# imironhead/ml_super_resolution

Hardware: AMD Instinct MI355X
Metric: VDSR-20 training patches/sec (41x41, batch 256 per GPU); fwd HR megapixels/sec alongside (higher is better)
Workload: dtype f32; 1 GPU; BASELINE configs[2]: VDSR 20-layer 3x3x64 residual, RGB, batch 256x41x41 per GPU, fwd+bwd+TF-Adam, random-init weights; global_batch=256, patch=41, parallelism=dp1

## Files before the change

### ml_super_resolution_amd/csrc/conv_narrow.hip

```cpp
#include "launchers.h"
namespace srx {
typedef float f32x3 __attribute__((ext_vector_type(3)));
typedef unsigned u32x3v __attribute__((ext_vector_type(3)));

template <int CTRL>
__device__ __forceinline__ float dpp_add(float v) {
    const int moved = __builtin_amdgcn_update_dpp(0, __float_as_int(v), CTRL, 0xf, 0xf, false);
    return v + __int_as_float(moved);
}

struct PixWalk {
    int n, oh, ow;
    __device__ __forceinline__ void init(unsigned p, int OH, int OW) {
        const unsigned t = p / (unsigned)OW;
        ow = (int)(p - t * (unsigned)OW);
        n = (int)(t / (unsigned)OH);
        oh = (int)(t - (unsigned)n * (unsigned)OH);
    }
    __device__ __forceinline__ void step16(int OH, int OW) { step(16, OH, OW); }
    __device__ __forceinline__ void step(int d, int OH, int OW) {
        ow += d;
        while (ow >= OW) {
            ow -= OW;
            oh += 1;
            if (oh == OH) { oh = 0; n += 1; }
        }
    }
};
template <int KH, int KW>
__device__ __forceinline__ void tap_offsets(int (&off)[KH * KW], const PixWalk& q, bool live, int H, int W, int pad_t, int pad_l,
                                            int PB, int lane_b) {
    const int centre = ((q.n * H + q.oh - pad_t) * W + (q.ow - pad_l)) * PB + lane_b;
    bool rok[KH], cok[KW];
#pragma unroll
    for (int kh = 0; kh < KH; ++kh) rok[kh] = live && (unsigned)(q.oh + kh - pad_t) < (unsigned)H;
#pragma unroll
    for (int kw = 0; kw < KW; ++kw) cok[kw] = (unsigned)(q.ow + kw - pad_l) < (unsigned)W;
#pragma unroll
    for (int kh = 0; kh < KH; ++kh)
#pragma unroll
        for (int kw = 0; kw < KW; ++kw)
            off[kh * KW + kw] = (rok[kh] && cok[kw]) ? centre + (kh * W + kw) * PB : kOobOffset;
}

template <int KH, int KW, int CIN, int CO>
__global__ __launch_bounds__(256) void conv_narrow_kernel(const ConvArgs a, long total_px, int iters) {
    static_assert(CIN == 64, "16 lanes x 4 channels per pixel");
    constexpr int TAPS = KH * KW;
    const int c4 = threadIdx.x & 15;
    const int sub = threadIdx.x >> 4;
    float wr[TAPS][4][CO];
#pragma unroll
    for (int t = 0; t < TAPS; ++t)
#pragma unroll
        for (int e = 0; e < 4; ++e)
#pragma unroll
            for (int c = 0; c < CO; ++c) wr[t][e][c] = a.w[((size_t)t * CIN + 4 * c4 + e) * CO + c];
    float bias[CO];
#pragma unroll
    for (int c = 0; c < CO; ++c) bias[c] = a.bias ? a.bias[c] : 0.0f;
    const __amdgpu_buffer_rsrc_t xrs = __builtin_amdgcn_make_buffer_rsrc(const_cast<float*>(a.x), 0,
                                                                         a.N * a.H * a.W * CIN * 4, 0x00020000);
    const unsigned p0 = blockIdx.x * (unsigned)iters * 16u + sub;
    PixWalk q;
    q.init(p0 < (unsigned)total_px ? p0 : 0u, a.OH, a.OW);
    for (int it = 0; it < iters; ++it, q.step16(a.OH, a.OW)) {
        const unsigned p = p0 + (unsigned)it * 16u;
        const bool live = p < (unsigned)total_px;
        int off[TAPS];
        tap_offsets<KH, KW>(off, q, live, a.H, a.W, a.pad_t, a.pad_l, CIN * 4, 16 * c4);
        f32x4 v[TAPS];
#pragma unroll
        for (int tp = 0; tp < TAPS; ++tp)
            v[tp] = __builtin_bit_cast(f32x4, __builtin_amdgcn_raw_buffer_load_b128(xrs, off[tp], 0, 0));
        float acc[CO];
#pragma unroll
        for (int c = 0; c < CO; ++c) acc[c] = 0.0f;
#pragma unroll
        for (int tp = 0; tp < TAPS; ++tp)
#pragma unroll
            for (int e = 0; e < 4; ++e)
#pragma unroll
                for (int c = 0; c < CO; ++c) acc[c] = fmaf(v[tp][e], wr[tp][e][c], acc[c]);
#pragma unroll
        for (int c = 0; c < CO; ++c) {
            float r = acc[c];
            r = dpp_add<0xB1>(r);
            r = dpp_add<0x4E>(r);
            r = dpp_add<0x124>(r);
            r = dpp_add<0x128>(r);
            acc[c] = r;
        }
        if (live && c4 < CO) {
            float r = (c4 == 0) ? acc[0] : (c4 == 1 ? acc[1 < CO ? 1 : 0] : acc[2 < CO ? 2 : 0]);
            r = act_apply(r + ((c4 == 0) ? bias[0] : (c4 == 1 ? bias[1 < CO ? 1 : 0] : bias[2 < CO ? 2 : 0])), a.act);
            const size_t o = (size_t)p * CO + c4;
            if (a.skip) r += a.skip[o];
            if (a.post_relu) r = act_apply(r, a.post_relu);
            a.y[o] = r;
        }
    }
}

template <int KH, int KW, bool NOUT, int CW = 64>
__global__ __launch_bounds__(256) void wgrad_narrow_kernel(const WgradArgs a, long total_px, int iters) {
    constexpr int TAPS = KH * KW, CN = 3;
    constexpr int LPP = CW / 4;
    constexpr int PPI = 256 / LPP;
    constexpr int NB = NOUT ? CN : 4;
    constexpr int NV = TAPS * 4 * CN + NB;
    __shared__ float red[4 * NV * LPP];
    const int c4 = threadIdx.x & (LPP - 1);
    const int sub = threadIdx.x / LPP;
    const int wave = threadIdx.x >> 6;
    float acc[NV];
#pragma unroll
    for (int i = 0; i < NV; ++i) acc[i] = 0.0f;
    const __amdgpu_buffer_rsrc_t xrs = __builtin_amdgcn_make_buffer_rsrc(
        const_cast<float*>(a.x), 0, a.N * a.H * a.W * (NOUT ? CW : CN) * 4, 0x00020000);
    const __amdgpu_buffer_rsrc_t drs = __builtin_amdgcn_make_buffer_rsrc(
        const_cast<float*>(a.dpre), 0, a.N * a.OH * a.OW * (NOUT ? CN : CW) * 4, 0x00020000);
    const unsigned p0 = blockIdx.x * (unsigned)iters * (unsigned)PPI + sub;
    PixWalk q;
    q.init(p0 < (unsigned)total_px ? p0 : 0u, a.OH, a.OW);
    for (int it = 0; it < iters; ++it, q.step(PPI, a.OH, a.OW)) {
        const unsigned p = p0 + (unsigned)it * (unsigned)PPI;
        const bool live = p < (unsigned)total_px;
        int off[TAPS];
        tap_offsets<KH, KW>(off, q, live, a.H, a.W, a.pad_t, a.pad_l, (NOUT ? CW : CN) * 4, NOUT ? 16 * c4 : 0);
        if constexpr (NOUT) {
            const f32x3 d = __builtin_bit_cast(f32x3, __builtin_amdgcn_raw_buffer_load_b96(drs, live ? (int)(p * CN * 4) : kOobOffset, 0, 0));
            f32x4 v[TAPS];
#pragma unroll
            for (int tp = 0; tp < TAPS; ++tp)
                v[tp] = __builtin_bit_cast(f32x4, __builtin_amdgcn_raw_buffer_load_b128(xrs, off[tp], 0, 0));
#pragma unroll
            for (int tp = 0; tp < TAPS; ++tp)
#pragma unroll
                for (int e = 0; e < 4; ++e)
#pragma unroll
                    for (int c = 0; c < CN; ++c) acc[(tp * 4 + e) * CN + c] = fmaf(v[tp][e], d[c], acc[(tp * 4 + e) * CN + c]);
#pragma unroll
            for (int c = 0; c < CN; ++c) acc[TAPS * 4 * CN + c] += d[c];
        } else {
            const f32x4 d = __builtin_bit_cast(f32x4, __builtin_amdgcn_raw_buffer_load_b128(
                drs, live ? (int)((p * CW + 4 * c4) * 4) : kOobOffset, 0, 0));
            f32x3 v[TAPS];
#pragma unroll
            for (int tp = 0; tp < TAPS; ++tp)
                v[tp] = __builtin_bit_cast(f32x3, __builtin_amdgcn_raw_buffer_load_b96(xrs, off[tp], 0, 0));
#pragma unroll
            for (int tp = 0; tp < TAPS; ++tp)
#pragma unroll
                for (int cn = 0; cn < CN; ++cn)
#pragma unroll
                    for (int e = 0; e < 4; ++e) acc[(tp * CN + cn) * 4 + e] = fmaf(v[tp][cn], d[e], acc[(tp * CN + cn) * 4 + e]);
#pragma unroll
            for (int e = 0; e < 4; ++e) acc[TAPS * 4 * CN + e] += d[e];
        }
    }
#pragma unroll
    for (int i = 0; i < NV; ++i) {
        float r = acc[i];
#pragma unroll
        for (int o = LPP; o < 64; o <<= 1) r += __shfl_xor(r, o);
        if (sub % (64 / LPP) == 0) red[(wave * NV + i) * LPP + c4] = r;
    }
    __syncthreads();
    float* part = a.part + (size_t)blockIdx.x * a.part_stride;
    const int wn = TAPS * CW * CN;
    for (int q = threadIdx.x; q < NV * LPP; q += 256) {
        const int i = q / LPP, l = q % LPP;
        const float r = (red[(0 * NV + i) * LPP + l] + red[(1 * NV + i) * LPP + l]) +
                        (red[(2 * NV + i) * LPP + l] + red[(3 * NV + i) * LPP + l]);
        if (i < TAPS * 4 * CN) {
            int idx;
            if constexpr (NOUT) {
                const int c = i % CN, te = i / CN, e = te & 3, tp = te >> 2;
                idx = (tp * CW + 4 * l + e) * CN + c;
            } else {
                const int e = i & 3, tc = i >> 2;
                idx = tc * CW + 4 * l + e;
            }
            part[idx] = r;
        } else {
            const int b = i - TAPS * 4 * CN;
            if constexpr (NOUT) {
                if (l == 0) part[wn + b] = r;
            } else {
                part[wn + 4 * l + b] = r;
            }
        }
    }
}

bool launch_wgrad_narrow(const ConvKey& k, const WgradArgs& a, int grid, hipStream_t s, hipError_t* err) {
    if (k.kh != 3 || k.kw != 3) return false;
    const bool nout = a.Cin == 64 && a.Cout == 3, nin = a.Cin == 3 && a.Cout == 64, nin32 = a.Cin == 3 && a.Cout == 32;
    if (!nout && !nin && !nin32) return false;
    const long total = (long)a.N * a.OH * a.OW;
    if (total >= (1L << 31) - 4096 || (long)a.N * a.H * a.W * 64 * 4 >= (1L << 31) - 4096 || total * 64 * 4 >= (1L << 31) - 4096)
        return false;
    const long ppi = nin32 ? 32 : 16;
    const int iters = (int)((total + ppi * grid - 1) / (ppi * grid));
    if (nout)
        hipLaunchKernelGGL((wgrad_narrow_kernel<3, 3, true>), dim3(grid), dim3(256), 0, s, a, total, iters);
    else if (nin)
        hipLaunchKernelGGL((wgrad_narrow_kernel<3, 3, false>), dim3(grid), dim3(256), 0, s, a, total, iters);
    else
        hipLaunchKernelGGL((wgrad_narrow_kernel<3, 3, false, 32>), dim3(grid), dim3(256), 0, s, a, total, iters);
    *err = hipGetLastError();
    return true;
}

bool launch_conv_narrow(const ConvKey& k, const ConvArgs& a, hipStream_t s, hipError_t* err) {
    if (k.wt || a.Cout != 3 || a.mask) return false;
    if ((long)a.N * a.H * a.W * a.Cin * 4 >= (1L << 31) - 4096) return false;
    const long total = (long)a.N * a.OH * a.OW;
    int iters = 16;
    while (iters > 1 && total / (16L * iters) < 2048) iters >>= 1;
    const long blocks = (total + 16L * iters - 1) / (16L * iters);
    if (total >= (1L << 31) - 4096) return false;
    if (k.kh == 3 && k.kw == 3 && a.Cin == 64) {
        hipLaunchKernelGGL((conv_narrow_kernel<3, 3, 64, 3>), dim3((unsigned)blocks), dim3(256), 0, s, a, total, iters);
    } else {
        return false;
    }
    *err = hipGetLastError();
    return true;
}
}
```

Before: 20200 patches/s.

## Add sliding-column walk kernel for narrow-channel 3x3 weight gradients

```diff
diff --git a/ml_super_resolution_amd/csrc/conv_narrow.hip b/ml_super_resolution_amd/csrc/conv_narrow.hip
--- a/ml_super_resolution_amd/csrc/conv_narrow.hip
+++ b/ml_super_resolution_amd/csrc/conv_narrow.hip
@@ -1,4 +1,5 @@
 #include "launchers.h"
+#include "narrow_walk.h"
 namespace srx {
 typedef float f32x3 __attribute__((ext_vector_type(3)));
 typedef unsigned u32x3v __attribute__((ext_vector_type(3)));
@@ -102,6 +103,53 @@
     }
 }
 
+template <int KH, int KW, bool NOUT, int CW, bool CE = false>
+__device__ __forceinline__ void wgrad_narrow_close(float (&acc)[KH * KW * 4 * 3 + (NOUT ? 3 : 4)], const WgradArgs& a, float* red) {
+    constexpr int TAPS = KH * KW, CN = 3;
+    constexpr int LPP = CW / 4;
+    constexpr int NB = NOUT ? CN : 4;
+    constexpr int NV = TAPS * 4 * CN + NB;
+    const int c4 = threadIdx.x & (LPP - 1);
+    const int sub = threadIdx.x / LPP;
+    const int wave = threadIdx.x >> 6;
+#pragma unroll
+    for (int i = 0; i < NV; ++i) {
+        float r = acc[i];
+#pragma unroll
+        for (int o = LPP; o < 64; o <<= 1) r += __shfl_xor(r, o);
+        if (sub % (64 / LPP) == 0) red[(wave * NV + i) * LPP + c4] = r;
+    }
+    __syncthreads();
+    float* part = a.part + (size_t)blockIdx.x * a.part_stride;
+    const int wn = TAPS * CW * CN;
+    for (int q = threadIdx.x; q < NV * LPP; q += 256) {
+        const int i = q / LPP, l = q % LPP;
+        const float r = (red[(0 * NV + i) * LPP + l] + red[(1 * NV + i) * LPP + l]) +
+                        (red[(2 * NV + i) * LPP + l] + red[(3 * NV + i) * LPP + l]);
+        if (i < TAPS * 4 * CN) {
+            int idx;
+            if constexpr (NOUT && CE) {
+                const int e = i & 3, tc = i >> 2, c = tc % CN, tp = tc / CN;
+                idx = (tp * CW + 4 * l + e) * CN + c;
+            } else if constexpr (NOUT) {
+                const int c = i % CN, te = i / CN, e = te & 3, tp = te >> 2;
+                idx = (tp * CW + 4 * l + e) * CN + c;
+            } else {
+                const int e = i & 3, tc = i >> 2;
+                idx = tc * CW + 4 * l + e;
+            }
+            part[idx] = r;
+        } else {
+            const int b = i - TAPS * 4 * CN;
+            if constexpr (NOUT) {
+                if (l == 0) part[wn + b] = r;
+            } else {
+                part[wn + 4 * l + b] = r;
+            }
+        }
+    }
+}
+
 template <int KH, int KW, bool NOUT, int CW = 64>
 __global__ __launch_bounds__(256) void wgrad_narrow_kernel(const WgradArgs a, long total_px, int iters) {
     constexpr int TAPS = KH * KW, CN = 3;
@@ -112,7 +160,6 @@
     __shared__ float red[4 * NV * LPP];
     const int c4 = threadIdx.x & (LPP - 1);
     const int sub = threadIdx.x / LPP;
-    const int wave = threadIdx.x >> 6;
     float acc[NV];
 #pragma unroll
     for (int i = 0; i < NV; ++i) acc[i] = 0.0f;
@@ -159,39 +206,116 @@
             for (int e = 0; e < 4; ++e) acc[TAPS * 4 * CN + e] += d[e];
         }
     }
-#pragma unroll
-    for (int i = 0; i < NV; ++i) {
-        float r = acc[i];
-#pragma unroll
-        for (int o = LPP; o < 64; o <<= 1) r += __shfl_xor(r, o);
-        if (sub % (64 / LPP) == 0) red[(wave * NV + i) * LPP + c4] = r;
-    }
-    __syncthreads();
-    float* part = a.part + (size_t)blockIdx.x * a.part_stride;
-    const int wn = TAPS * CW * CN;
-    for (int q = threadIdx.x; q < NV * LPP; q += 256) {
-        const int i = q / LPP, l = q % LPP;
-        const float r = (red[(0 * NV + i) * LPP + l] + red[(1 * NV + i) * LPP + l]) +
-                        (red[(2 * NV + i) * LPP + l] + red[(3 * NV + i) * LPP + l]);
-        if (i < TAPS * 4 * CN) {
-            int idx;
+    wgrad_narrow_close<KH, KW, NOUT, CW>(acc, a, red);
+}
+
+#ifndef SRX_WGRAD_WALK_DEPTH_OUT
+#define SRX_WGRAD_WALK_DEPTH_OUT 2
+#endif
+#ifndef SRX_WGRAD_WALK_DEPTH_IN
+#define SRX_WGRAD_WALK_DEPTH_IN 1
+#endif
+constexpr int kWalkDepthOut = SRX_WGRAD_WALK_DEPTH_OUT, kWalkDepthIn = SRX_WGRAD_WALK_DEPTH_IN;
+template <bool NOUT, int D, int PAD>
+__global__ __launch_bounds__(256, 2) void wgrad_narrow_walk_kernel(const WgradArgs a, unsigned total, int iters) {
+    constexpr int KH = 3, KW = 3, TAPS = KH * KW, CN = 3, CW = 64, LPP = CW / 4;
+    constexpr int U = D + KW;
+    constexpr int NB = NOUT ? CN : 4;
+    constexpr int NV = TAPS * 4 * CN + NB;
+    __shared__ float red[4 * NV * LPP];
+    const int c4 = threadIdx.x & (LPP - 1);
+    const int sub = threadIdx.x / LPP;
+    float acc[NV];
+#pragma unroll
+    for (int i = 0; i < NV; ++i) acc[i] = 0.0f;
+    const int Hw = NOUT ? a.H : a.OH, Ww = NOUT ? a.W : a.OW, Hn = NOUT ? a.OH : a.H, Wn = NOUT ? a.OW : a.W;
+    const float* wide_p = NOUT ? a.x : a.dpre;
+    const float* narrow_p = NOUT ? a.dpre : a.x;
+    const __amdgpu_buffer_rsrc_t wrs = __builtin_amdgcn_make_buffer_rsrc(const_cast<float*>(wide_p), 0, a.N * Hw * Ww * CW * 4, 0x00020000);
+    const __amdgpu_buffer_rsrc_t nrs = __builtin_amdgcn_make_buffer_rsrc(const_cast<float*>(narrow_p), 0, a.N * Hn * Wn * CN * 4, 0x00020000);
+    const int coff = NOUT ? a.pad_l : KW - 1 - a.pad_l;
+    const int Wn12 = Wn * CN * 4;
+    int roff[KH], roffb[KH];
+#pragma unroll
+    for (int r = 0; r < KH; ++r) { roff[r] = NOUT ? a.pad_t - r : r - a.pad_t; roffb[r] = roff[r] * Wn12; }
+
+    const int cur_row = Wn12 - (Ww + KW - 2) * (CN * 4), cur_image = cur_row + (Hn - Hw) * Wn12;
+    const NarrowRun run = narrow_run(total, gridDim.x, 256 / LPP, blockIdx.x, (unsigned)sub);
+    int left = (int)(run.end - run.begin);
+    int row, vc, c_lo, woff, cur;
+    {
+        const unsigned p = left > 0 ? run.begin : 0u;
+        const unsigned t = p / (unsigned)Ww, col = p - t * (unsigned)Ww, n = t / (unsigned)Hw;
+        row = (int)(t - n * (unsigned)Hw);
+        c_lo = (int)col;
+        vc = c_lo - (KW - 1);
+        woff = (int)(p * (unsigned)(CW * 4)) + 16 * c4;
+        cur = ((int)n * Hn + row) * Wn12 + (vc + coff) * (CN * 4);
+    }
+    f32x3 colv[U][KH];
+    unsigned lives = 0;
+    f32x4 wide[U];
+#pragma unroll
+    for (int k = 0; k < U; ++k) {
+        wide[k] = f32x4{0.0f, 0.0f, 0.0f, 0.0f};
+#pragma unroll
+        for (int r = 0; r < KH; ++r) colv[k][r] = f32x3{0.0f, 0.0f, 0.0f};
+    }
+    auto issue = [&](f32x3 (&cv)[KH], f32x4& wv) {
+        const bool alive = left > 0;
+        const bool live = alive & (vc >= c_lo);
+        const int nc = vc + coff;
+        const bool cok = alive & ((unsigned)nc < (unsigned)Wn);
+#pragma unroll
+        for (int r = 0; r < KH; ++r) {
+            const bool ok = cok & ((unsigned)(row + roff[r]) < (unsigned)Hn);
+            cv[r] = __builtin_bit_cast(f32x3, __builtin_amdgcn_raw_buffer_load_b96(nrs, ok ? cur + roffb[r] : kOobOffset, 0, 0));
+        }
+        wv = __builtin_bit_cast(f32x4, __builtin_amdgcn_raw_buffer_load_b128(wrs, live ? woff : kOobOffset, 0, 0));
+        if constexpr (NOUT) lives = (lives << 1) | (live ? 1u : 0u);
+        woff += live ? CW * 4 : 0;
+        left -= live ? 1 : 0;
+        const bool wrap = vc + 1 == Ww;
+        const bool iwrap = wrap & (row + 1 == Hw);
+        vc = wrap ? -(KW - 1) : vc + 1;
+        c_lo = wrap ? 0 : c_lo;
+        row = iwrap ? 0 : row + (wrap ? 1 : 0);
+        cur += wrap ? (iwrap ? cur_image : cur_row) : CN * 4;
+    };
+#pragma unroll
+    for (int k = 0; k < D; ++k) issue(colv[k], wide[k]);
+    for (int it = 0; it < iters; ++it) {
+#pragma unroll
+        for (int u = 0; u < U; ++u) {
+            issue(colv[(u + D) % U], wide[(u + D) % U]);
+            __builtin_amdgcn_sched_barrier(0);
+            const f32x4 d = wide[u];
+#pragma unroll
+            for (int j = 0; j < KW; ++j) {
+                const int sl = (u + U - j) % U, kw = NOUT ? j : KW - 1 - j;
+#pragma unroll
+                for (int r = 0; r < KH; ++r) {
+                    const int tp = r * KW + kw;
+                    const f32x3 v = colv[sl][r];
+#pragma unroll
+                    for (int cn = 0; cn < CN; ++cn)
+#pragma unroll
+                        for (int e = 0; e < 4; ++e) acc[(tp * CN + cn) * 4 + e] = fmaf(v[cn], d[e], acc[(tp * CN + cn) * 4 + e]);
+                }
+            }
             if constexpr (NOUT) {
-                const int c = i % CN, te = i / CN, e = te & 3, tp = te >> 2;
-                idx = (tp * CW + 4 * l + e) * CN + c;
+                const float m = (float)((lives >> D) & 1u);
+#pragma unroll
+                for (int c = 0; c < CN; ++c)
+                    acc[TAPS * 4 * CN + c] = fmaf(m, colv[(u + U - PAD) % U][PAD][c], acc[TAPS * 4 * CN + c]);
             } else {
-                const int e = i & 3, tc = i >> 2;
-                idx = tc * CW + 4 * l + e;
+#pragma unroll
+                for (int e = 0; e < 4; ++e) acc[TAPS * 4 * CN + e] += d[e];
             }
-            part[idx] = r;
-        } else {
-            const int b = i - TAPS * 4 * CN;
-            if constexpr (NOUT) {
-                if (l == 0) part[wn + b] = r;
-            } else {
-                part[wn + 4 * l + b] = r;
-            }
-        }
-    }
+            __builtin_amdgcn_sched_barrier(0);
+        }
+    }
+    wgrad_narrow_close<KH, KW, NOUT, CW, true>(acc, a, red);
 }
 
 bool launch_wgrad_narrow(const ConvKey& k, const WgradArgs& a, int grid, hipStream_t s, hipError_t* err) {
@@ -201,14 +325,24 @@
     const long total = (long)a.N * a.OH * a.OW;
     if (total >= (1L << 31) - 4096 || (long)a.N * a.H * a.W * 64 * 4 >= (1L << 31) - 4096 || total * 64 * 4 >= (1L << 31) - 4096)
         return false;
-    const long ppi = nin32 ? 32 : 16;
-    const int iters = (int)((total + ppi * grid - 1) / (ppi * grid));
-    if (nout)
+    if (nin32) {
+        const int iters = (int)((total + 32L * grid - 1) / (32L * grid));
+        hipLaunchKernelGGL((wgrad_narrow_kernel<3, 3, false, 32>), dim3(grid), dim3(256), 0, s, a, total, iters);
+    } else if (nout && (a.pad_t != a.pad_l || a.pad_t < 0 || a.pad_t > 1)) {
+        const int iters = (int)((total + 16L * grid - 1) / (16L * grid));
         hipLaunchKernelGGL((wgrad_narrow_kernel<3, 3, true>), dim3(grid), dim3(256), 0, s, a, total, iters);
-    else if (nin)
-        hipLaunchKernelGGL((wgrad_narrow_kernel<3, 3, false>), dim3(grid), dim3(256), 0, s, a, total, iters);
-    else
-        hipLaunchKernelGGL((wgrad_narrow_kernel<3, 3, false, 32>), dim3(grid), dim3(256), 0, s, a, total, iters);
+    } else {
+        const int D = nout ? kWalkDepthOut : kWalkDepthIn;
+        const unsigned walked = (unsigned)(nout ? (long)a.N * a.H * a.W : total), width = (unsigned)(nout ? a.W : a.OW);
+        const unsigned steps = narrow_walk_steps(narrow_run_len(walked, (unsigned)grid, 16), width, 2);
+        const int iters = (int)((steps + D + 2) / (D + 3));
+        if (nout && a.pad_t == 1)
+            hipLaunchKernelGGL((wgrad_narrow_walk_kernel<true, kWalkDepthOut, 1>), dim3(grid), dim3(256), 0, s, a, walked, iters);
+        else if (nout)
+            hipLaunchKernelGGL((wgrad_narrow_walk_kernel<true, kWalkDepthOut, 0>), dim3(grid), dim3(256), 0, s, a, walked, iters);
+        else
+            hipLaunchKernelGGL((wgrad_narrow_walk_kernel<false, kWalkDepthIn, 0>), dim3(grid), dim3(256), 0, s, a, walked, iters);
+    }
     *err = hipGetLastError();
     return true;
 }
diff --git a/ml_super_resolution_amd/csrc/narrow_walk.h b/ml_super_resolution_amd/csrc/narrow_walk.h
--- /dev/null
+++ b/ml_super_resolution_amd/csrc/narrow_walk.h
@@ -0,0 +1,36 @@
+#pragma once
+#if defined(__HIPCC__) || defined(__CUDACC__)
+#define SRX_NARROW_HD __host__ __device__
+#else
+#define SRX_NARROW_HD
+#endif
+
+namespace srx {
+
+struct NarrowRun {
+    unsigned begin, end;
+};
+
+SRX_NARROW_HD inline unsigned narrow_wg_len(unsigned total, unsigned grid) { return total / grid + (total % grid != 0); }
+SRX_NARROW_HD inline unsigned narrow_run_len(unsigned total, unsigned grid, unsigned groups) {
+    const unsigned c = narrow_wg_len(total, grid);
+    return c / groups + (c % groups != 0);
+}
+
+SRX_NARROW_HD inline NarrowRun narrow_run(unsigned total, unsigned grid, unsigned groups, unsigned block, unsigned group) {
+    const unsigned long long c = narrow_wg_len(total, grid), r = narrow_run_len(total, grid, groups);
+    unsigned long long wb = c * block, we = wb + c;
+    if (wb > total) wb = total;
+    if (we > total) we = total;
+    unsigned long long b = wb + r * group, e = b + r;
+    if (b > we) b = we;
+    if (e > we) e = we;
+    NarrowRun run = {(unsigned)b, (unsigned)e};
+    return run;
+}
+
+SRX_NARROW_HD inline unsigned narrow_walk_steps(unsigned len, unsigned width, unsigned lead) {
+    return len ? len + lead * ((len + 2 * width - 2) / width) : 0;
+}
+
+}
```

Measured after the change: 20290 patches/s (median of 6 runs). About the same (+0.4%).
